# LiWentomng/OrientedRepPoints

Hardware: AMD Instinct MI355X
Metric: images/sec (1024x1024 DOTA, R-50 FPN) (higher is better)
Workload: dtype f32; 1 GPU; configs[1]: OrientedRepPoints R-50 FPN inference, 1024x1024 patch, 15 classes, bs=1/GPU, nms_pre=2000, score_thr=0.05, rnms iou_thr=0.4, max_per_img=2000; random-init weights, head biases calibrated to ~2000 dets/img; global_batch=1, parallelism=replicas x1 (image-parallel, no collective), images_in_flight_per_gpu=4

## Files before the change

include/orp_hip.h:

```cpp
#ifndef ORP_HIP_H_
#define ORP_HIP_H_

#include <stddef.h>
#include <stdint.h>

#ifdef __cplusplus
extern "C" {
#endif

#define ORP_OK 0
#define ORP_EINVAL (-1)
#define ORP_EWORKSPACE (-2)
#define ORP_ETOOBIG (-3)

const char* orp_version(void);

#define ORP_NMS_MAX_BOXES 131072
size_t orp_rnms_workspace_bytes(int n);
int orp_rnms(const float* dets, int n, float iou_thr, int flavor, int presorted, int order_out,
             int64_t* keep_out, int32_t* num_keep, void* workspace, size_t workspace_bytes, void* stream);

size_t orp_rnms_batched_workspace_bytes(int n_total, int nseg, int max_seg);
int orp_rnms_batched(const float* dets, int n_total, const int32_t* seg_offsets, int nseg, int max_seg,
                     float iou_thr, int flavor, int64_t* keep_out, int32_t* num_keep,
// ... 239 lines not shown
int orp_affine2_act(const float* x, const float* residual, const float* scale, const float* shift, const float* scale2,
                    const float* shift2, float* y, int batch, int channels, int hw, int relu, void* stream);
int orp_affine_relu_maxpool(const float* x, const float* scale, const float* shift, float* y, int batch, int channels,
                            int height, int width, void* stream);
size_t orp_affine_act_backward_workspace_bytes(int batch, int channels, int hw);
int orp_affine_act_backward(const float* grad_y, const float* y, const float* x, const float* scale, const float* mean,
                            const float* rstd, float* grad_x, float* grad_res, float* dweight, float* dbias, int batch, int channels,
                            int hw, void* workspace, size_t workspace_bytes, void* stream);
int orp_affine2_act_backward(const float* grad_y, const float* y, const float* x, const float* scale, const float* mean,
                             const float* rstd, const float* x2, const float* scale2, const float* mean2, const float* rstd2,
                             float* grad_x, float* grad_x2, float* grad_res, float* dweight, float* dbias, float* dweight2,
                             float* dbias2, int batch, int channels, int hw, void* workspace, size_t workspace_bytes, void* stream);
size_t orp_fpn_topdown_workspace_bytes(const orp_norm_level* levels, int nlevels, int batch, int channels, int groups);
int orp_fpn_topdown_nhwc(const orp_norm_level* levels, const float* const* gammas_host, const float* const* betas_host,
                         int nlevels, int batch, int channels, int groups, float eps, uint32_t* amax_out, void* workspace,
                         size_t workspace_bytes, void* stream);

typedef struct { const float* input; const float* residual; float* output; float* output2; int height; int width; } orp_bias_level;
int orp_bias_act_multi(const orp_bias_level* levels_host, int nlevels, int batch, int channels, const float* bias,
                       const float* sub, int relu, void* stream);

size_t orp_conv1x1_packed_floats(int c_in);
int orp_conv1x1_ok(int c_in, int c_out);
int orp_conv1x1_pack_weight(const float* weight, int c_out, int c_in, float* packed, void* stream);
int orp_conv1x1_multi(const orp_bias_level* levels_host, int nlevels, int batch, int c_in, int c_out,
                      const float* weight_packed, const float* bias, const float* sub, int relu, void* stream);

int orp_conv1x1_bn_act_ok(int c_in, int c_out);
int orp_conv1x1_bn_act_pays(int c_in, int c_out, int hw, int batch, int has_residual);
int orp_conv1x1_bn_act_tile(int c_in, int c_out, int hw, int batch, int* tile_channels, int* tile_positions);
int orp_conv1x1_bn_act(const float* x, const float* weight_t, const float* scale, const float* shift, const float* residual,
                       const float* scale2, const float* shift2, float* y, int batch, int c_in, int c_out, int hw, int relu,
                       void* stream);

int orp_conv1x1_bn_act_range(const float* x, const float* weight_t, const float* scale, const float* shift, const float* residual,
                             const float* scale2, const float* shift2, float* y, int batch, int c_in, int c_out, int hw, int relu,
                             uint32_t* range_out, void* stream);
int orp_conv1x1_bn_act_pieces_ok(int c_in, int c_out);
int orp_conv1x1_bn_act_pieces_pays(int c_in, int c_out, int hw, int batch, int has_residual);
int orp_conv1x1_bn_act_pieces_tile(int c_in, int c_out, int hw, int batch, int* tile_channels, int* tile_positions);
size_t orp_conv1x1_bn_pieces_packed_bytes(int c_in, int c_out);
int orp_conv1x1_bn_pieces_pack_weight(const float* weight, int c_in, int c_out, void* packed, void* stream);
int orp_conv1x1_bn_act_pieces(const float* x, const void* weight_packed, const float* scale, const float* shift,
                              const float* residual, const float* scale2, const float* shift2, float* y, int batch, int c_in,
                              int c_out, int hw, int relu, uint32_t* range_out, void* stream);

int orp_conv1x1_bn_act_pieces_dual_ok(int c_in, int c_in2, int c_out);
int orp_conv1x1_bn_act_pieces_dual_pays(int c_in, int c_in2, int c_out, int hw, int stride2, int batch);
int orp_conv1x1_bn_act_pieces_dual_tile(int c_in, int c_in2, int c_out, int hw, int batch, int* tile_channels, int* tile_positions);
int orp_conv1x1_bn_act_pieces_dual(const float* x, const void* w_packed, const float* scale, const float* shift, const float* x2,
                                   const void* w2_packed, const float* scale2, const float* shift2, int c_in2, int h2, int w2,
                                   int stride2, float* y, int batch, int c_in, int c_out, int ho, int wo, int relu, void* stream);

int orp_affine_act_range(const float* x, const float* residual, const float* scale, const float* shift, float* y, int batch,
                         int channels, int hw, int relu, uint32_t* range_out, void* stream);

int orp_conv3x3_bn_act_ok(int c_in, int c_out);
int orp_conv3x3_bn_act_pays(int c_in, int c_out, int height, int width, int batch);
int orp_conv3x3_bn_act_tile(int c_in, int c_out, int height, int width, int batch, int* tile_h, int* tile_w, int* waves_pos,
                            int* waves_ch);
size_t orp_conv3x3_bn_packed_bytes(int c_in, int c_out);
int orp_conv3x3_bn_pack_weight(const float* weight, int c_in, int c_out, void* packed, void* stream);
int orp_conv3x3_bn_act(const float* x, const void* weight_packed, const float* scale, const float* shift, const uint32_t* range_in,
                       float* y, int batch, int c_in, int c_out, int height, int width, int relu, void* stream);

int orp_conv3x3_bn_deep_ok(int c_in, int c_out, int stride);
int orp_conv3x3_bn_deep_pays(int c_in, int c_out, int height, int width, int stride, int batch);
size_t orp_conv3x3_bn_deep_packed_bytes(int c_in, int c_out);
int orp_conv3x3_bn_deep_pack_weight(const float* weight, int c_in, int c_out, void* packed, void* stream);
int orp_conv3x3_bn_deep(const float* x, const void* weight_packed, const float* scale, const float* shift, const uint32_t* range_in,
                        float* y, int batch, int c_in, int c_out, int height, int width, int stride, int relu, void* stream);

int orp_conv3x3_bn_s2_ok(int c_in, int c_out);
int orp_conv3x3_bn_s2_pays(int c_in, int c_out, int height, int width, int batch);
size_t orp_conv3x3_bn_s2_packed_bytes(int c_in, int c_out);
int orp_conv3x3_bn_s2_pack_weight(const float* weight, int c_in, int c_out, void* packed, void* stream);
int orp_conv3x3_bn_s2(const float* x, const void* weight_packed, const float* scale, const float* shift, const uint32_t* range_in,
                      float* y, int batch, int c_in, int c_out, int height, int width, int relu, void* stream);

int orp_stem_ok(int c_in, int c_out, int kernel, int stride, int padding);
int orp_stem_pays(int height, int width, int batch);
size_t orp_stem_packed_bytes(int c_in, int c_out);
int orp_stem_pack_weight(const float* weight, int c_in, int c_out, void* packed, void* stream);
int orp_stem_conv_bn_relu_pool(const float* x, const void* weight_packed, const float* scale, const float* shift, float* y, int batch,
                               int c_in, int c_out, int height, int width, int kernel, int stride, int padding, int pool, void* stream);


int orp_conv3x3_small_ok(int c_in, int c_out);
int orp_conv3x3_small_multi(const orp_norm_level* levels_host, int nlevels, int batch, int c_in, int c_out,
                            const float* weight_packed, void* stream);
int orp_conv3x3_small_multi_ex(const orp_norm_level* levels_host, const float* const* weights_packed_host, int nlevels,
                               int batch, int c_in, int c_out, void* stream);
size_t orp_conv3x3_small_workspace_bytes(const orp_norm_level* levels_host, const int* strides_host, int nlevels, int batch,
                                         int c_out);
int orp_conv3x3_small_multi_strided(const orp_norm_level* levels_host, const float* const* weights_packed_host,
                                    const int* strides_host, int nlevels, int batch, int c_in, int c_out, void* workspace,
                                    size_t workspace_bytes, void* stream);

typedef struct { const float* input_a; const float* input_b; float* output_a; float* output_b; int height; int width; } orp_conv_level;
int orp_conv_split_ok(int c_in, int c_out, int kh, int kw);
int orp_conv_split_multi(const orp_conv_level* levels_host, int nlevels, int batch, int c_in, int c_out,
                         const float* weight_a_packed, const float* weight_b_packed, const float* bias_a, const float* bias_b,
                         int relu, int kh, int kw, int stride_h, int stride_w, int pad_h, int pad_w, int dil_h, int dil_w,
                         int out_layout, int nprod, void* workspace, size_t workspace_bytes, const uint32_t* amax_in,
                         int amax_stride, void* stream);
int orp_conv_split_multi_ex(const orp_conv_level* levels_host, const float* const* weights_packed_host,
// ... 88 lines not shown
```

orientedreppoints_amd/build.py:

```python
import concurrent.futures
import os
import subprocess

HERE = os.path.dirname(os.path.abspath(__file__))
CSRC = os.path.join(HERE, "csrc")
LIB = os.path.join(CSRC, "liborp_hip.so")
HIPCC = os.environ.get("HIPCC", "/opt/rocm/bin/hipcc")
ARCH = "gfx950"

NO_PACKED_FP32 = ["-Xclang", "-target-feature", "-Xclang", "-packed-fp32-ops"]
COMMON = ["--offload-arch=" + ARCH, "-O3", "-std=c++17", "-fPIC", "-Wall", "-Wno-unused-function",
          "-Wno-unused-result", "-Wno-unused-value",
          "-Wno-bitwise-instead-of-logical"]
if os.environ.get("ORP_PACKED_FP32", "0") != "1":
    COMMON = COMMON + NO_PACKED_FP32
SOURCES = [
    ("orp_nms.hip", ["-ffp-contract=off"]),
    ("orp_overlaps.hip", ["-ffp-contract=off"]),
    ("orp_minarearect.hip", ["-ffp-contract=off"]),
    ("orp_box_iou_rotated.hip", ["-ffp-contract=off"]),
    ("orp_convex.hip", ["-ffp-contract=off"]),
    ("orp_convex_giou.hip", ["-ffp-contract=off"]),
    ("orp_pointwise.hip", ["-ffp-contract=off"]),
    ("orp_assign.hip", ["-ffp-contract=off"]),
    ("orp_postproc.hip", ["-ffp-contract=off"]),
    ("orp_soft_rnms.hip", ["-ffp-contract=off"]),
    ("orp_scene.hip", ["-ffp-contract=off"]),
    ("orp_train_images.hip", ["-ffp-contract=off"]),
    ("orp_eval.hip", ["-ffp-contract=off"]),
    ("orp_train.hip", ["-ffp-contract=off"]),
    ("orp_norm.hip", []),
    ("orp_conv_small.hip", []),
    ("orp_conv1x1.hip", []),
    ("orp_conv1x1_bn.hip", []),
    ("orp_conv1x1_bn_pieces.hip", []),
    ("orp_conv3x3_bn.hip", []),
    ("orp_conv3x3_bn_deep.hip", []),
    ("orp_conv3x3_bn_s2.hip", []),
    ("orp_stem.hip", []),
    ("orp_dcn.hip", []),
    ("orp_dcn_split.hip", ["-ffp-contract=off"]),
    ("orp_conv_split.hip", []),
    ("orp_conv_wgrad.hip", []),
    ("orp_dcn_half.hip", []),
    ("orp_dcn_bwd.hip", []),
    ("orp_dcn_bwd_mfma.hip", []),
    ("orp_window_attn.hip", []),
    ("orp_token_linear.hip", []),
    ("orp_prof.hip", []),
]
HEADERS = sorted(f for f in os.listdir(CSRC) if f.endswith(".hpp")) + [os.path.join("..", "..", "include", "orp_hip.h")]


def _stale(target, deps):
    if not os.path.exists(target):
        return True
    t = os.path.getmtime(target)
    return any(os.path.getmtime(d) > t for d in deps if os.path.exists(d))


VERSION_SOURCE = "orp_overlaps.hip"


def build_id():
    import hashlib
    h = hashlib.sha1()
    names = sorted([s for s, _ in SOURCES] + [x for x in HEADERS])
    for n in names:
        path = os.path.join(CSRC, n)
        if os.path.exists(path):
            h.update(n.encode())
            h.update(open(path, "rb").read())
    return h.hexdigest()[:12]


def _compile(src, extra):
    obj = os.path.join(CSRC, os.path.splitext(src)[0] + ".o")
    deps = [os.path.join(CSRC, src)] + [os.path.join(CSRC, h) for h in HEADERS] + [os.path.abspath(__file__)]
    if src == VERSION_SOURCE:
        deps += [os.path.join(CSRC, s) for s, _ in SOURCES]
        extra = extra + ['-DORP_BUILD_ID="%s"' % build_id()]
    if _stale(obj, deps):
        cmd = [HIPCC] + COMMON + extra + ["-c", os.path.join(CSRC, src), "-o", obj]
        r = subprocess.run(cmd, cwd=CSRC, stderr=subprocess.PIPE, universal_newlines=True)
        err = "\n".join(l for l in r.stderr.splitlines() if "'-packed-fp32-ops' is not a recognized feature" not in l)
        if err.strip():
            import sys
            sys.stderr.write(err + "\n")
# ... 27 lines not shown
```

orientedreppoints_amd/mmdet_models/resnet.py:

```python
import functools

import torch
import torch.nn as nn

from .. import switches
from .layers import build_conv_layer, build_norm_layer, constant_init, kaiming_init
from .registry import BACKBONES


class Bottleneck(nn.Module):
    expansion = 4

    def __init__(self, inplanes, planes, stride=1, dilation=1, downsample=None, style='pytorch',
                 norm_cfg=dict(type='BN'), dcn=None):
        super(Bottleneck, self).__init__()
        assert style in ['pytorch', 'caffe']
        assert dcn is None or isinstance(dcn, dict)
        if style == 'pytorch':
            conv1_stride, conv2_stride = 1, stride
        else:
            conv1_stride, conv2_stride = stride, 1
        self.conv1 = nn.Conv2d(inplanes, planes, kernel_size=1, stride=conv1_stride, bias=False)
        self.add_module('bn1', build_norm_layer(norm_cfg, planes)[1])
        self.with_dcn = dcn is not None
# ... 19 lines not shown
            isinstance(self.bn1, nn.BatchNorm2d) and not self.bn1.training and not self.bn3.training

    def _norms_are_eval_bn(self):
        return all(isinstance(bn, nn.BatchNorm2d) and not bn.training for bn in (self.bn1, self.bn2, self.bn3)) and \
            (self.downsample is None or self._downsample_is_conv_norm())

    def _frozen_ok(self, x):
        return torch.is_grad_enabled() and not torch.is_autocast_enabled() and x.is_cuda and x.dtype == torch.float32 and \
            not x.requires_grad and not getattr(self, 'with_cp', False) and \
            isinstance(self.bn1, nn.BatchNorm2d) and not self.bn1.training and not self.bn3.training and \
            switches.of(self, 'fuse_bn_frozen', 'BN_FROZEN_FUSE') and not any(p.requires_grad for p in self.parameters())

    def _train_fused_ok(self, x):
        return torch.is_grad_enabled() and not torch.is_autocast_enabled() and x.is_cuda and x.dtype == torch.float32 and \
            x.dim() == 4 and x.is_contiguous() and not getattr(self, 'with_cp', False) and self._norms_are_eval_bn() and \
            switches.of(self, 'fuse_bn_train', 'BN_TRAIN_FUSE')

    def route(self, x):
        if self._fused_ok(x):
            return 'fused'
        if self._frozen_ok(x):
            return 'frozen'
        if self._train_fused_ok(x):
            return 'train'
        return 'stock'

    def _forward_train_fused(self, x):
        from ..mmdet_ops.fused_norm import bn_act_train
        out = bn_act_train(self.conv1(x).contiguous(), self.bn1, relu=True)
        out = bn_act_train(self.conv2(out).contiguous(), self.bn2, relu=True)
        out = self.conv3(out).contiguous()
        ds = self.downsample
        if ds is not None:
            return bn_act_train(out, self.bn3, residual=ds[0](x).contiguous(), residual_bn=ds[1], relu=True)
        return bn_act_train(out, self.bn3, residual=x, relu=True)

    def _downsample_norm_fusable(self):
        return switches.of(self, 'fuse_downsample_norm', 'BN_DOWNSAMPLE_FUSE') and self._downsample_is_conv_norm()

    def _downsample_is_conv_norm(self):
        ds = self.downsample
        return isinstance(ds, nn.Sequential) and len(ds) == 2 and isinstance(ds[0], nn.Conv2d) and \
            isinstance(ds[1], nn.BatchNorm2d) and not ds[1].training

    def _conv1x1_fusable(self):
        return switches.of(self, 'fuse_conv1x1', 'BN_CONV1X1_FUSE')

    def _conv1x1_pieces_on(self):
        return switches.of(self, 'fuse_conv1x1_pieces', 'BN_CONV1X1_PIECES')

    def _downsample_conv_fusable(self):
        return switches.of(self, 'fuse_downsample_conv', 'BN_DOWNSAMPLE_CONV_FUSE')

    def _conv3x3_fusable(self, kind='act'):
        from ..mmdet_ops.fused_norm import conv3x3_kernel
        k = conv3x3_kernel(kind)
        return switches.of(self, k.fuse_attr, k.switch) and not self.conv2_is_dcn and \
            isinstance(self.bn2, nn.BatchNorm2d) and not self.bn2.training

    _conv3x3_deep_fusable = functools.partialmethod(_conv3x3_fusable, 'deep')
    _conv3x3_s2_fusable = functools.partialmethod(_conv3x3_fusable, 's2')

    def _conv3x3_forced(self, kind):
        from ..mmdet_ops.fused_norm import conv3x3_kernel
        return bool(getattr(self, conv3x3_kernel(kind).force_attr, False))

    def _forward_fused(self, x):
        from ..mmdet_ops.fused_norm import bn_act, conv1x1_bn_act, conv3x3_bn_route, _conv3x3_launch, conv1x1_bn_act_dual, \
            conv1x1_bn_act_dual_routed
        fuse = self._conv1x1_fusable()
        pieces = None if self._conv1x1_pieces_on() else False

        def conv_bn_act(t, conv, bn, **kw):
            if fuse:
                return conv1x1_bn_act(t, conv, bn, pieces=pieces, **kw)
            return bn_act(conv(t).contiguous(), bn, **kw)
        kind = None
        if tuple(self.conv1.stride) == (1, 1):
            kind = conv3x3_bn_route(x, self.conv2, self.bn2, (x.size(0), self.conv1.out_channels, x.size(2), x.size(3)),
                                    self._conv3x3_fusable, self._conv3x3_forced)
        if kind is not None:
            out, bits = conv_bn_act(x, self.conv1, self.bn1, relu=True, want_range=True)
            out = _conv3x3_launch(kind, out, self.conv2, self.bn2, relu=True, force=self._conv3x3_forced(kind), range_bits=bits)
        else:
            out = conv_bn_act(x, self.conv1, self.bn1, relu=True)
            out = bn_act(self.conv2(out).contiguous(), self.bn2, relu=True)
        ds = self.downsample
        if fuse and pieces is None and self._downsample_conv_fusable() and self._downsample_is_conv_norm() and \
                conv1x1_bn_act_dual_routed(out, self.conv3, self.bn3, x, ds[0], ds[1]):
            return conv1x1_bn_act_dual(out, self.conv3, self.bn3, x, ds[0], ds[1], relu=True)
        if self._downsample_norm_fusable():
            residual, residual_bn = ds[0](x).contiguous(), ds[1]
        elif ds is not None:
            residual, residual_bn = bn_act(ds[0](x).contiguous(), ds[1], relu=False), None
        else:
            residual, residual_bn = x.contiguous(), None
        return conv_bn_act(out, self.conv3, self.bn3, residual=residual, residual_bn=residual_bn, relu=True)

    def forward(self, x):
        route = self.route(x)
        if route == 'fused':
            return self._forward_fused(x)
        if route == 'frozen':
            with torch.no_grad():
                return self._forward_fused(x)
        if route == 'train':
            return self._forward_train_fused(x)
        identity = x
        out = self.relu(self.bn1(self.conv1(x)))
        out = self.relu(self.bn2(self.conv2(out)))
        out = self.bn3(self.conv3(out))
        if self.downsample is not None:
            identity = self.downsample(x)
        out += identity
        return self.relu(out)


@BACKBONES.register_module
class ResNet(nn.Module):
    arch_settings = {50: (Bottleneck, (3, 4, 6, 3)), 101: (Bottleneck, (3, 4, 23, 3)), 152: (Bottleneck, (3, 8, 36, 3))}

    def __init__(self, depth, in_channels=3, num_stages=4, strides=(1, 2, 2, 2), dilations=(1, 1, 1, 1),
                 out_indices=(0, 1, 2, 3), style='pytorch', frozen_stages=-1, conv_cfg=None,
                 norm_cfg=dict(type='BN', requires_grad=True), norm_eval=True, dcn=None,
                 stage_with_dcn=(False, False, False, False), gcb=None, stage_with_gcb=None, gen_attention=None,
                 stage_with_gen_attention=None, with_cp=False, zero_init_residual=True):
        super(ResNet, self).__init__()
        if depth not in self.arch_settings:
            raise KeyError('invalid depth {} for resnet'.format(depth))
        assert gcb is None and gen_attention is None, 'context / attention blocks are not part of the DOTA configs'
        assert conv_cfg is None, 'the backbone convolutions are stock nn.Conv2d (dcn= selects the deformable conv2)'
        self.dcn = dict(dcn) if dcn is not None else None
        self.stage_with_dcn = tuple(stage_with_dcn) if stage_with_dcn is not None else (False,) * num_stages
        if dcn is not None:
            assert len(self.stage_with_dcn) == num_stages
        self.depth, self.num_stages, self.out_indices = depth, num_stages, out_indices
        self.frozen_stages, self.norm_eval = frozen_stages, norm_eval
        self.zero_init_residual = zero_init_residual
        block, stage_blocks = self.arch_settings[depth]
        self.conv1 = nn.Conv2d(in_channels, 64, kernel_size=7, stride=2, padding=3, bias=False)
        self.add_module('bn1', build_norm_layer(norm_cfg, 64)[1])
        self.relu = nn.ReLU(inplace=True)
        self.maxpool = nn.MaxPool2d(kernel_size=3, stride=2, padding=1)
        inplanes = 64
        self.res_layers = []
        for i, num_blocks in enumerate(stage_blocks[:num_stages]):
            planes = 64 * 2 ** i
            stride, dilation = strides[i], dilations[i]
            downsample = None
            if stride != 1 or inplanes != planes * block.expansion:
                downsample = nn.Sequential(
                    nn.Conv2d(inplanes, planes * block.expansion, kernel_size=1, stride=stride, bias=False),
                    build_norm_layer(norm_cfg, planes * block.expansion)[1])
            stage_dcn = self.dcn if (self.dcn is not None and self.stage_with_dcn[i]) else None
            layers = [block(inplanes, planes, stride, dilation, downsample, style, norm_cfg, stage_dcn)]
            inplanes = planes * block.expansion
            for _ in range(1, num_blocks):
                layers.append(block(inplanes, planes, 1, dilation, None, style, norm_cfg, stage_dcn))
# ... 32 lines not shown
                if missing or unexpected:
                    warnings.warn('ResNet.init_weights(%r): missing keys %s, unexpected keys %s'
                                  % (pretrained, list(missing)[:8], unexpected[:8]))
                return
            warnings.warn('ResNet.init_weights: pretrained=%r was NOT loaded (no such file%s); the backbone keeps its '
                          'random initialisation, frozen_stages=%d of it frozen'
                          % (pretrained, '' if '://' not in pretrained else '; set ORP_PRETRAINED_DIR', self.frozen_stages))
        for m in self.modules():
            if isinstance(m, nn.Conv2d):
                kaiming_init(m)
            elif isinstance(m, (nn.BatchNorm2d, nn.GroupNorm)):
                constant_init(m, 1)
        if self.dcn is not None:
            for m in self.modules():
                if isinstance(m, Bottleneck) and hasattr(m.conv2, 'conv_offset'):
                    constant_init(m.conv2.conv_offset, 0)
        if self.zero_init_residual:
            for m in self.modules():
                if isinstance(m, Bottleneck):
                    constant_init(m.bn3, 0)

    def _stem_pool_fusable(self):
        from ..mmdet_ops.fused_norm import is_maxpool_3_2_1
        return switches.of(self, 'fuse_stem_pool', 'STEM_POOL_FUSE') and is_maxpool_3_2_1(self.maxpool)

    def stem_route(self, x):
        if not (x.is_cuda and x.dtype == torch.float32 and isinstance(self.bn1, nn.BatchNorm2d) and not self.bn1.training):
            return 'stock'
        if not torch.is_grad_enabled():
            return 'fused'
        if not torch.is_autocast_enabled() and not x.requires_grad and switches.of(self, 'fuse_bn_frozen', 'BN_FROZEN_FUSE') and \
                not any(p.requires_grad for m in (self.conv1, self.bn1) for p in m.parameters()):
            return 'frozen'
        return 'stock'

    def _forward_stem_fused(self, x):
        from ..mmdet_ops.fused_norm import bn_act, bn_relu_maxpool, stem_conv_bn_relu_maxpool, stem_conv_routed
        if switches.of(self, 'fuse_stem_conv', 'STEM_CONV_FUSE') and \
                stem_conv_routed(x, self.conv1, self.bn1, self.maxpool, bool(getattr(self, 'force_stem_conv', False))):
            return stem_conv_bn_relu_maxpool(x, self.conv1, self.bn1)
        if self._stem_pool_fusable():
            return bn_relu_maxpool(self.conv1(x).contiguous(), self.bn1)
        return self.maxpool(bn_act(self.conv1(x).contiguous(), self.bn1, relu=True))

    def forward(self, x):
        route = self.stem_route(x)
        if route == 'fused':
            x = self._forward_stem_fused(x)
        elif route == 'frozen':
            with torch.no_grad():
                x = self._forward_stem_fused(x)
        else:
            x = self.maxpool(self.relu(self.bn1(self.conv1(x))))
        outs = []
        for i, name in enumerate(self.res_layers):
            x = getattr(self, name)(x)
            if i in self.out_indices:
                outs.append(x)
        return tuple(outs)

    def train(self, mode=True):
        super(ResNet, self).train(mode)
        self._freeze_stages()
        if mode and self.norm_eval:
            for m in self.modules():
                if isinstance(m, nn.modules.batchnorm._BatchNorm):
                    m.eval()
```

orientedreppoints_amd/mmdet_ops/fused_norm.py:

```python
import collections
import ctypes
import functools

import torch

from .. import _lib, _packcache


_NormLevel = _lib.struct("orp_norm_level")


def _call(name, device, *args):
    with torch.cuda.device(device):
        rc = getattr(_lib.lib(), name)(*args)
    _lib.check(rc, name)


def _norm_levels(ins, outs):
    levels = (_NormLevel * len(ins))()
    for i, (x, y) in enumerate(zip(ins, outs)):
        levels[i] = _NormLevel(x.data_ptr(), y.data_ptr() if y is not None else None, x.size(2), x.size(3))
    return levels


# ... 238 lines not shown
    y = torch.empty((B, cout, H, W), dtype=torch.float32, device=x.device)
    bits = torch.empty(1, dtype=torch.int32, device=x.device) if want_range else None
    args = (_lib.ptr(x), _lib.ptr(weight), _lib.ptr(scale), _lib.ptr(shift), _lib.ptr(residual), _lib.ptr(scale2), _lib.ptr(shift2),
            _lib.ptr(y), B, cin, cout, H * W, 1 if relu else 0)
    if route == 'pieces':
        _call("orp_conv1x1_bn_act_pieces", x.device, *args, _lib.ptr(bits), _lib.stream_of(x))
    elif want_range:
        _call("orp_conv1x1_bn_act_range", x.device, *args, _lib.ptr(bits), _lib.stream_of(x))
    else:
        _call("orp_conv1x1_bn_act", x.device, *args, _lib.stream_of(x))
    return (y, bits) if want_range else y


def conv1x1_bn_act_dual_ok(x, conv, bn, x2, conv2, bn2):
    if not conv1x1_bn_act_ok(x, conv, bn):
        return False
    w2 = getattr(conv2, 'weight', None)
    if not (isinstance(conv2, torch.nn.Conv2d) and _bn_input(x2, bn2) and x2.dim() == 4 and x2.device == x.device and
            _plain_conv(conv2, w2, 1, ((1, 1), (2, 2)), 0) and x2.size(1) == w2.size(1) and
            w2.size(0) == conv.weight.size(0) and x2.size(0) == x.size(0)):
        return False
    s = conv2.stride[0]
    return bool(x2.size(2) > 0 and x2.size(3) > 0 and (x2.size(2) - 1) // s + 1 == x.size(2) and (x2.size(3) - 1) // s + 1 == x.size(3)
                and _lib.lib().orp_conv1x1_bn_act_pieces_dual_ok(conv.weight.size(1), w2.size(1), w2.size(0)))


def conv1x1_bn_act_dual_pays(x, conv, x2, conv2):
    return bool(_lib.lib().orp_conv1x1_bn_act_pieces_dual_pays(conv.weight.size(1), conv2.weight.size(1), conv.weight.size(0),
                                                               x.size(2) * x.size(3), conv2.stride[0], x.size(0)))


def conv1x1_bn_act_dual_routed(x, conv, bn, x2, conv2, bn2):
    return conv1x1_bn_act_dual_ok(x, conv, bn, x2, conv2, bn2) and conv1x1_bn_act_dual_pays(x, conv, x2, conv2)


def conv1x1_bn_act_dual_tile(cin, cin2, cout, hw, B):
    return _tile_query("orp_conv1x1_bn_act_pieces_dual_tile", 2, cin, cin2, cout, hw, B)


def conv1x1_bn_act_dual(x, conv, bn, x2, conv2, bn2, relu=True):
    if not conv1x1_bn_act_dual_ok(x, conv, bn, x2, conv2, bn2):
        raise ValueError("conv1x1_bn_act_dual: unsupported modules or shapes (conv1x1_bn_act_dual_ok)")
    x, x2 = x.detach().contiguous(), x2.detach().contiguous()
    B, cin, H, W = x.shape
    cout, cin2 = conv.weight.size(0), conv2.weight.size(1)
    packed, packed2 = _packed_1x1_planes(conv.weight), _packed_1x1_planes(conv2.weight)
    scale, shift = _bn_affine(bn)
    scale2, shift2 = _bn_affine(bn2)
    y = torch.empty((B, cout, H, W), dtype=torch.float32, device=x.device)
    _call("orp_conv1x1_bn_act_pieces_dual", x.device, _lib.ptr(x), _lib.ptr(packed), _lib.ptr(scale), _lib.ptr(shift), _lib.ptr(x2),
          _lib.ptr(packed2), _lib.ptr(scale2), _lib.ptr(shift2), cin2, x2.size(2), x2.size(3), conv2.stride[0], _lib.ptr(y),
          B, cin, cout, H, W, 1 if relu else 0, _lib.stream_of(x))
    return y


_Conv3x3Kernel = collections.namedtuple("_Conv3x3Kernel", "kind strides ok pays packed_bytes pack_weight launch takes_stride "
                                                           "switch fuse_attr force_attr")
CONV3X3_KERNELS = (
    _Conv3x3Kernel("act", ((1, 1),), "orp_conv3x3_bn_act_ok", "orp_conv3x3_bn_act_pays", "orp_conv3x3_bn_packed_bytes",
                   "orp_conv3x3_bn_pack_weight", "orp_conv3x3_bn_act", False, "BN_CONV3X3_FUSE", "fuse_conv3x3", "force_conv3x3"),
    _Conv3x3Kernel("deep", ((1, 1), (2, 2)), "orp_conv3x3_bn_deep_ok", "orp_conv3x3_bn_deep_pays", "orp_conv3x3_bn_deep_packed_bytes",
                   "orp_conv3x3_bn_deep_pack_weight", "orp_conv3x3_bn_deep", True, "BN_CONV3X3_DEEP_FUSE", "fuse_conv3x3_deep",
                   "force_conv3x3_deep"),
    _Conv3x3Kernel("s2", ((2, 2),), "orp_conv3x3_bn_s2_ok", "orp_conv3x3_bn_s2_pays", "orp_conv3x3_bn_s2_packed_bytes",
                   "orp_conv3x3_bn_s2_pack_weight", "orp_conv3x3_bn_s2", False, "BN_CONV3X3_S2_FUSE", "fuse_conv3x3_s2", "force_conv3x3_s2"),
)
_CONV3X3 = {k.kind: k for k in CONV3X3_KERNELS}


def conv3x3_kernel(kind):
    return _CONV3X3[kind]


def _stride_arg(k, conv):
    return (conv.stride[0],) if k.takes_stride else ()


def _conv3x3_ok(kind, x, conv, bn, shape=None):
    k = _CONV3X3[kind]
    w = getattr(conv, 'weight', None)
    shape = tuple(x.shape) if shape is None else tuple(shape)
    return bool(type(conv) is torch.nn.Conv2d and _bn_input(x, bn) and len(shape) == 4 and
                _plain_conv(conv, w, 3, k.strides, 1) and shape[1] == w.size(1) and shape[0] * shape[2] * shape[3] > 0 and
                getattr(_lib.lib(), k.ok)(w.size(1), w.size(0), *_stride_arg(k, conv)))


def _conv3x3_routed(kind, x, conv, bn, force=False, shape=None):
    if not _conv3x3_ok(kind, x, conv, bn, shape):
        return False
    k = _CONV3X3[kind]
    B, _c, H, W = tuple(x.shape) if shape is None else tuple(shape)
    return bool(force or getattr(_lib.lib(), k.pays)(conv.weight.size(1), conv.weight.size(0), H, W, *_stride_arg(k, conv), B))


def conv3x3_bn_route(x, conv, bn, shape, enabled, forced):
    for k in CONV3X3_KERNELS:
        if enabled(k.kind) and _conv3x3_routed(k.kind, x, conv, bn, forced(k.kind), shape):
            return k.kind
    return None


_packed_3x3_cache = _packcache.new_cache("conv3x3_bn_weight")


def _packed_3x3(kind, weight):
    k = _CONV3X3[kind]
# ... 800 lines not shown
```

orientedreppoints_amd/switches.py:

```python
import os


def _on(name, default='1'):
    return os.environ.get(name, default) == '1'


TOWER_SPLIT = _on('ORP_TOWER_SPLIT')
FPN_SPLIT = _on('ORP_FPN_SPLIT')
TOWER_GN_FUSE = _on('ORP_TOWER_GN_FUSE')
BN_DOWNSAMPLE_FUSE = _on('ORP_BN_DOWNSAMPLE_FUSE')
BN_CONV1X1_FUSE = _on('ORP_BN_CONV1X1_FUSE')
BN_CONV1X1_PIECES = _on('ORP_BN_CONV1X1_PIECES')
BN_DOWNSAMPLE_CONV_FUSE = _on('ORP_BN_DOWNSAMPLE_CONV_FUSE')
BN_CONV3X3_FUSE = _on('ORP_BN_CONV3X3_FUSE')
BN_CONV3X3_DEEP_FUSE = _on('ORP_BN_CONV3X3_DEEP_FUSE')
BN_CONV3X3_S2_FUSE = _on('ORP_BN_CONV3X3_S2_FUSE')
BN_TRAIN_FUSE = _on('ORP_BN_TRAIN_FUSE')
BN_FROZEN_FUSE = _on('ORP_BN_FROZEN_FUSE')
STEM_POOL_FUSE = _on('ORP_STEM_POOL_FUSE')
STEM_CONV_FUSE = _on('ORP_STEM_CONV_FUSE')
SWIN_ATTN_FUSE = _on('ORP_SWIN_ATTN_FUSE')
SWIN_ATTN_TRAIN_FUSE = _on('ORP_SWIN_ATTN_TRAIN_FUSE')
SWIN_ATTN_HALF_FUSE = _on('ORP_SWIN_ATTN_HALF_FUSE')
SWIN_LINEAR_FUSE = _on('ORP_SWIN_LINEAR_FUSE')
FPN_TOPDOWN_FUSE = _on('ORP_FPN_TOPDOWN_FUSE')
TRAIN_SPLIT = _on('ORP_TRAIN_SPLIT')
DETERMINISTIC = _on('ORP_DETERMINISTIC', '0')


def of(obj, attr, name):
    on = getattr(obj, attr, None)
    return bool(globals()[name] if on is None else on)
```

Baseline: 468.0 images/s.

## Fuse bottleneck conv3 with next block's conv1 in one chained 1x1 kernel

Adds a HIP kernel that computes a bottleneck's final 1x1 conv+BN+residual+ReLU and immediately feeds the result tile from LDS into the next block's first 1x1 conv+BN+ReLU, writing both outputs. The ResNet forward links consecutive Bottleneck blocks so the next block reuses the handed-off conv1 output and range bits. This removes one kernel launch and the re-read of the wide intermediate from global memory for the second conv. It is gated by a pays table covering only the 128->512->128 stage-2 shape at hw=16384, batch 1. It adds per-forward Python bookkeeping and a new MFMA kernel with a heavier LDS and register footprint.

```diff
diff --git a/include/orp_hip.h b/include/orp_hip.h
--- a/include/orp_hip.h
+++ b/include/orp_hip.h
@@ -315,6 +315,14 @@
                                    const void* w2_packed, const float* scale2, const float* shift2, int c_in2, int h2, int w2,
                                    int stride2, float* y, int batch, int c_in, int c_out, int ho, int wo, int relu, void* stream);
 
+int orp_conv1x1_bn_act_pieces_chain_ok(int c_in, int c_out, int c_next);
+int orp_conv1x1_bn_act_pieces_chain_pays(int c_in, int c_out, int c_next, int hw, int batch);
+int orp_conv1x1_bn_act_pieces_chain_tile(int c_in, int c_out, int c_next, int hw, int batch, int* tile_channels, int* tile_positions);
+int orp_conv1x1_bn_act_pieces_chain(const float* x, const void* w_packed, const float* scale, const float* shift, const float* residual,
+                                    float* y, const void* w_next_packed, const float* scale_next, const float* shift_next, float* t,
+                                    int batch, int c_in, int c_out, int c_next, int hw, int relu, int relu_next, uint32_t* range_out,
+                                    void* stream);
+
 int orp_affine_act_range(const float* x, const float* residual, const float* scale, const float* shift, float* y, int batch,
                          int channels, int hw, int relu, uint32_t* range_out, void* stream);
 
diff --git a/orientedreppoints_amd/build.py b/orientedreppoints_amd/build.py
--- a/orientedreppoints_amd/build.py
+++ b/orientedreppoints_amd/build.py
@@ -34,6 +34,7 @@
     ("orp_conv1x1.hip", []),
     ("orp_conv1x1_bn.hip", []),
     ("orp_conv1x1_bn_pieces.hip", []),
+    ("orp_conv1x1_bn_chain.hip", []),
     ("orp_conv3x3_bn.hip", []),
     ("orp_conv3x3_bn_deep.hip", []),
     ("orp_conv3x3_bn_s2.hip", []),
diff --git a/orientedreppoints_amd/csrc/orp_conv1x1_bn_chain.hip b/orientedreppoints_amd/csrc/orp_conv1x1_bn_chain.hip
--- /dev/null
+++ b/orientedreppoints_amd/csrc/orp_conv1x1_bn_chain.hip
@@ -0,0 +1,372 @@
+#include <hip/hip_runtime.h>
+#include <stdint.h>
+
+#include "../../include/orp_hip.h"
+#include "orp_affine.hpp"
+#include "orp_range.hpp"
+#include "orp_launch.hpp"
+#include "orp_conv1x1_bn_host.hpp"
+#include "orp_dcn_split.hpp"
+
+namespace {
+
+constexpr int kThreads = 256;
+constexpr int kTileCh = 128;
+constexpr int kMaxCout = 1024;
+
+typedef float f32x16 __attribute__((ext_vector_type(16)));
+typedef __bf16 bf8 __attribute__((ext_vector_type(8)));
+
+struct ChainArgs {
+  const float* x;
+  const uint16_t* planes;
+  size_t plane_stride;
+  const float* scale; const float* shift;
+  const float* res;
+  float* y;
+  const uint16_t* planes2;
+  size_t plane_stride2;
+  const float* scale2; const float* shift2;
+  float* t;
+  int cout, hw, relu, relu2;
+  int ntn;
+  int vec;
+  unsigned* range;
+};
+
+using orp_split::split_pair;
+
+__device__ __forceinline__ void six(f32x16& acc, const bf8 (&w)[3], const bf8 (&x)[3]) {
+  acc = __builtin_amdgcn_mfma_f32_32x32x16_bf16(w[0], x[2], acc, 0, 0, 0);
+  acc = __builtin_amdgcn_mfma_f32_32x32x16_bf16(w[2], x[0], acc, 0, 0, 0);
+  acc = __builtin_amdgcn_mfma_f32_32x32x16_bf16(w[1], x[1], acc, 0, 0, 0);
+  acc = __builtin_amdgcn_mfma_f32_32x32x16_bf16(w[0], x[1], acc, 0, 0, 0);
+  acc = __builtin_amdgcn_mfma_f32_32x32x16_bf16(w[1], x[0], acc, 0, 0, 0);
+  acc = __builtin_amdgcn_mfma_f32_32x32x16_bf16(w[0], x[0], acc, 0, 0, 0);
+}
+
+constexpr size_t chain_lds_bytes(int cin, int bn) {
+  return (size_t)3 * bn * (cin + 8 + kTileCh + 8) * 2 + (size_t)2 * kTileCh * 4;
+}
+
+template <int CIN, int CNEXT, int WN>
+__global__ void __launch_bounds__(kThreads, 2)
+conv1x1_bn_chain_kernel(const ChainArgs P) {
+  constexpr int BN = 32 * WN;
+  constexpr int XSTR = CIN + 8, YSTR = kTileCh + 8;
+  constexpr int XPLANE = BN * XSTR, YPLANE = BN * YSTR;
+  constexpr int NCH = CIN / 16;
+  constexpr int NCH2 = kTileCh / 16;
+  constexpr int WCH2 = CNEXT >= 128 ? 4 : 2, WPOS2 = 4 / WCH2;
+  constexpr int MT2 = CNEXT / (32 * WCH2), NT2 = WN / WPOS2;
+  static_assert(NT2 >= 1 && MT2 >= 1, "Cnext = 64 needs 64 positions");
+  constexpr int D1 = MT2 * NT2 >= 4 ? 2 : 3;
+  constexpr int D2 = MT2 == 1 ? 4 : 2;
+  constexpr int ITEMS = (CIN / 2) * (BN / 4);
+  constexpr int XV = ITEMS / kThreads;
+  static_assert(ITEMS % kThreads == 0, "whole trips");
+
+  extern __shared__ __align__(16) uint16_t lds[];
+  uint16_t* Xs = lds;
+  uint16_t* Ys = lds + 3 * XPLANE;
+  float* Cs = reinterpret_cast<float*>(Ys + 3 * YPLANE);
+
+  const int tid = threadIdx.x;
+  const int nt = blockIdx.x % P.ntn, b = blockIdx.x / P.ntn;
+  const int p0 = nt * BN;
+  const int hw = P.hw, cout = P.cout;
+  const float* xb = P.x + (size_t)b * CIN * hw;
+
+  const int lane = tid & 63, wave = tid >> 6;
+  const int kg = lane >> 5, l31 = lane & 31;
+
+  const size_t plane0 = (size_t)b * cout;
+  float rv[WN][16];
+  auto load_res = [&](int m0) {
+#pragma unroll
+    for (int ni = 0; ni < WN; ni++) {
+      const int p = min(p0 + 32 * ni + l31, hw - 1);
+#pragma unroll
+      for (int r = 0; r < 16; r++) {
+        const int ch = m0 + 32 * wave + 8 * (r >> 2) + 4 * kg + (r & 3);
+        rv[ni][r] = P.res[(plane0 + ch) * hw + p];
+      }
+    }
+  };
+
+  {
+    float4 xr[XV][2];
+#pragma unroll
+    for (int i = 0; i < XV; i++) {
+      const int idx = tid + i * kThreads;
+      const int pq = idx % (BN / 4), kp = idx / (BN / 4);
+      const int col = p0 + 4 * pq;
+#pragma unroll
+      for (int h = 0; h < 2; h++) {
+        const float* src = xb + (size_t)(2 * kp + h) * hw;
+        if (P.vec) {
+          xr[i][h] = *reinterpret_cast<const float4*>(src + min(col, hw - 4));
+        } else {
+          xr[i][h].x = src[min(col, hw - 1)]; xr[i][h].y = src[min(col + 1, hw - 1)];
+          xr[i][h].z = src[min(col + 2, hw - 1)]; xr[i][h].w = src[min(col + 3, hw - 1)];
+        }
+      }
+    }
+#pragma unroll
+    for (int i = 0; i < XV; i++) {
+      const int idx = tid + i * kThreads;
+      const int pq = idx % (BN / 4), kp = idx / (BN / 4);
+      const int col = p0 + 4 * pq;
+      float v[2][4];
+#pragma unroll
+      for (int h = 0; h < 2; h++) {
+        v[h][0] = col < hw ? xr[i][h].x : 0.f; v[h][1] = col + 1 < hw ? xr[i][h].y : 0.f;
+        v[h][2] = col + 2 < hw ? xr[i][h].z : 0.f; v[h][3] = col + 3 < hw ? xr[i][h].w : 0.f;
+      }
+      const int rot = (pq >> 1) & 3;
+#pragma unroll
+      for (int h = 0; h < 2; h++) {
+        if (rot & 1) { const float t0 = v[h][0]; v[h][0] = v[h][1]; v[h][1] = v[h][2]; v[h][2] = v[h][3]; v[h][3] = t0; }
+        if (rot & 2) { const float t0 = v[h][0], t1 = v[h][1]; v[h][0] = v[h][2]; v[h][1] = v[h][3]; v[h][2] = t0; v[h][3] = t1; }
+      }
+      unsigned* base = reinterpret_cast<unsigned*>(Xs) + kp;
+#pragma unroll
+      for (int j = 0; j < 4; j++) {
+        unsigned d[3];
+        split_pair(v[0][j], v[1][j], d);
+        unsigned* dst = base + (4 * pq + ((j + rot) & 3)) * (XSTR / 2);
+#pragma unroll
+        for (int pl = 0; pl < 3; pl++) dst[pl * (XPLANE / 2)] = d[pl];
+      }
+    }
+  }
+
+  const size_t ps = P.plane_stride, ps2 = P.plane_stride2;
+  const size_t wblk = (size_t)2 * cout * 8, wblk2 = (size_t)2 * CNEXT * 8;
+  const uint16_t* wp = P.planes + ((size_t)kg * cout + 32 * wave + l31) * 8;
+  const int wc2 = (wave / WPOS2) * 32 * MT2, wn2 = (wave % WPOS2) * 32 * NT2;
+  const uint16_t* wp2 = P.planes2 + ((size_t)kg * CNEXT + wc2 + l31) * 8;
+  bf8 wq[NCH][3], w2q[NCH2][MT2][3];
+  auto load_w = [&](int m0, int c) {
+    const uint16_t* a = wp + (size_t)m0 * 8 + (size_t)c * wblk;
+#pragma unroll
+    for (int pl = 0; pl < 3; pl++) wq[c][pl] = *reinterpret_cast<const bf8*>(a + (size_t)pl * ps);
+  };
+  auto load_w2 = [&](int chunk0, int c) {
+    const uint16_t* a = wp2 + (size_t)(chunk0 + c) * wblk2;
+#pragma unroll
+    for (int mi = 0; mi < MT2; mi++)
+#pragma unroll
+      for (int pl = 0; pl < 3; pl++) w2q[c][mi][pl] = *reinterpret_cast<const bf8*>(a + (size_t)pl * ps2 + (size_t)mi * 32 * 8);
+  };
+
+  f32x16 tacc[MT2][NT2];
+#pragma unroll
+  for (int mi = 0; mi < MT2; mi++)
+#pragma unroll
+    for (int ni = 0; ni < NT2; ni++)
+#pragma unroll
+      for (int r = 0; r < 16; r++) tacc[mi][ni][r] = 0.f;
+
+#pragma unroll
+  for (int c = 0; c < D1; c++) load_w(0, c);
+  __syncthreads();
+
+  const int ntm = cout / kTileCh;
+  const uint16_t* xa = Xs + l31 * XSTR + 8 * kg;
+  const uint16_t* ya = Ys + (wn2 + l31) * YSTR + 8 * kg;
+  for (int mt = 0; mt < ntm; mt++) {
+    const int m0 = mt * kTileCh;
+    if (tid < kTileCh) { Cs[tid] = P.scale[m0 + tid]; Cs[kTileCh + tid] = P.shift[m0 + tid]; }
+    load_res(m0);
+    f32x16 acc[WN];
+#pragma unroll
+    for (int ni = 0; ni < WN; ni++)
+#pragma unroll
+      for (int r = 0; r < 16; r++) acc[ni][r] = 0.f;
+    __builtin_amdgcn_sched_barrier(0);
+
+#pragma unroll
+    for (int c = 0; c < NCH; c++) {
+      bf8 xq[WN][3];
+#pragma unroll
+      for (int ni = 0; ni < WN; ni++)
+#pragma unroll
+        for (int pl = 0; pl < 3; pl++) xq[ni][pl] = *reinterpret_cast<const bf8*>(xa + pl * XPLANE + ni * 32 * XSTR + c * 16);
+#pragma unroll
+      for (int ni = 0; ni < WN; ni++) six(acc[ni], wq[c], xq[ni]);
+      __builtin_amdgcn_sched_barrier(0);
+      if (c + D1 < NCH) load_w(m0, c + D1);
+      __builtin_amdgcn_sched_barrier(0);
+    }
+#pragma unroll
+    for (int c = 0; c < D2; c++) load_w2(mt * NCH2, c);
+    __builtin_amdgcn_sched_barrier(0);
+    __syncthreads();
+
+#pragma unroll
+    for (int g = 0; g < 4; g++) {
+      const int chl = 32 * wave + 8 * g + 4 * kg;
+      const float4 a4 = *reinterpret_cast<const float4*>(Cs + chl);
+      const float4 b4 = *reinterpret_cast<const float4*>(Cs + kTileCh + chl);
+      const float av[4] = {a4.x, a4.y, a4.z, a4.w}, bv[4] = {b4.x, b4.y, b4.z, b4.w};
+#pragma unroll
+      for (int ni = 0; ni < WN; ni++) {
+        const int pl_ = 32 * ni + l31, p = p0 + pl_;
+        float v[4];
+#pragma unroll
+        for (int q = 0; q < 4; q++) {
+          v[q] = affine_res_act(acc[ni][4 * g + q], av[q], bv[q], rv[ni][4 * g + q], P.relu);
+          if (p < hw) P.y[(plane0 + m0 + chl + q) * hw + p] = v[q];
+        }
+        unsigned d0[3], d1[3];
+        split_pair(v[0], v[1], d0);
+        split_pair(v[2], v[3], d1);
+        uint2* dst = reinterpret_cast<uint2*>(Ys + pl_ * YSTR + chl);
+#pragma unroll
+        for (int pl = 0; pl < 3; pl++) dst[pl * (YPLANE / 4)] = make_uint2(d0[pl], d1[pl]);
+      }
+    }
+    __builtin_amdgcn_sched_barrier(0);
+#pragma unroll
+    for (int c = 0; c < D1; c++) load_w(min(mt + 1, ntm - 1) * kTileCh, c);
+    __syncthreads();
+
+#pragma unroll
+    for (int c = 0; c < NCH2; c++) {
+      bf8 yq[NT2][3];
+#pragma unroll
+      for (int ni = 0; ni < NT2; ni++)
+#pragma unroll
+        for (int pl = 0; pl < 3; pl++) yq[ni][pl] = *reinterpret_cast<const bf8*>(ya + pl * YPLANE + ni * 32 * YSTR + c * 16);
+#pragma unroll
+      for (int mi = 0; mi < MT2; mi++)
+#pragma unroll
+        for (int ni = 0; ni < NT2; ni++) six(tacc[mi][ni], w2q[c][mi], yq[ni]);
+      __builtin_amdgcn_sched_barrier(0);
+      if (c + D2 < NCH2) load_w2(mt * NCH2, c + D2);
+      __builtin_amdgcn_sched_barrier(0);
+    }
+  }
+
+  unsigned rmax = 0u;
+  const size_t tplane0 = (size_t)b * CNEXT;
+#pragma unroll
+  for (int mi = 0; mi < MT2; mi++)
+#pragma unroll
+    for (int g = 0; g < 4; g++) {
+      const int ch = wc2 + 32 * mi + 8 * g + 4 * kg;
+      float av[4], bv[4];
+#pragma unroll
+      for (int q = 0; q < 4; q++) { av[q] = P.scale2[ch + q]; bv[q] = P.shift2[ch + q]; }
+#pragma unroll
+      for (int ni = 0; ni < NT2; ni++) {
+        const int p = p0 + wn2 + 32 * ni + l31;
+#pragma unroll
+        for (int q = 0; q < 4; q++) {
+          const float v = affine_act(tacc[mi][ni][4 * g + q], av[q], bv[q], P.relu2);
+          if (p < hw) {
+            P.t[(tplane0 + ch + q) * hw + p] = v;
+            rmax = max(rmax, orp::range_bits(v));
+          }
+        }
+      }
+    }
+  if (P.range) {
+#pragma unroll
+    for (int o = 32; o > 0; o >>= 1) rmax = max(rmax, (unsigned)__shfl_xor((int)rmax, o, 64));
+    unsigned* red = reinterpret_cast<unsigned*>(lds);
+    __syncthreads();
+    if (lane == 0) red[wave] = rmax;
+    __syncthreads();
+    if (tid == 0) orp::range_raise(P.range, max(max(red[0], red[1]), max(red[2], red[3])));
+  }
+}
+
+int pick_bn(int c_next, int hw, int batch) {
+  if (c_next < 128) return 64;
+  return (long)((hw + 63) / 64) * batch >= 256 ? 64 : 32;
+}
+
+template <int CIN, int CNEXT, int WN>
+hipError_t launch(const ChainArgs& A, int batch, hipStream_t st) {
+  const size_t smem = chain_lds_bytes(CIN, 32 * WN);
+  struct Tag {};
+  hipError_t e = orp::set_max_dynamic_lds_once<Tag>(reinterpret_cast<const void*>(&conv1x1_bn_chain_kernel<CIN, CNEXT, WN>), smem);
+  if (e != hipSuccess) return e;
+  hipLaunchKernelGGL((conv1x1_bn_chain_kernel<CIN, CNEXT, WN>), dim3((unsigned)((long)A.ntn * batch)), dim3(kThreads), smem, st, A);
+  return hipGetLastError();
+}
+
+bool overlap(const void* a, size_t na, const void* b, size_t nb) {
+  const uintptr_t x = (uintptr_t)a, y = (uintptr_t)b;
+  return x < y + nb && y < x + na;
+}
+
+}
+
+extern "C" {
+
+int orp_conv1x1_bn_act_pieces_chain_ok(int c_in, int c_out, int c_next) {
+  const bool pair = (c_in == 64 && (c_next == 64 || c_next == 128)) || (c_in == 128 && (c_next == 128 || c_next == 256));
+  return (pair && c_out >= kTileCh && c_out <= kMaxCout && c_out % kTileCh == 0) ? 1 : 0;
+}
+
+int orp_conv1x1_bn_act_pieces_chain_tile(int c_in, int c_out, int c_next, int hw, int batch, int* tile_channels, int* tile_positions) {
+  if (!orp_conv1x1_bn_act_pieces_chain_ok(c_in, c_out, c_next) || hw <= 0 || batch <= 0) return 0;
+  if (tile_channels) *tile_channels = c_out;
+  if (tile_positions) *tile_positions = pick_bn(c_next, hw, batch);
+  return 1;
+}
+
+int orp_conv1x1_bn_act_pieces_chain_pays(int c_in, int c_out, int c_next, int hw, int batch) {
+  if (!orp_conv1x1_bn_act_pieces_chain_ok(c_in, c_out, c_next) || hw <= 0 || batch <= 0) return 0;
+  if (!orp_conv1x1_bn_act_pieces_pays(c_in, c_out, hw, batch, 1) || !orp_conv1x1_bn_act_pieces_pays(c_out, c_next, hw, batch, 0)) return 0;
+  static const struct { int cin, cout, cnext, hw_min, hw_max, batch; } paid[] = {
+      {128, 512, 128, 16384, 16384, 1},
+  };
+  for (const auto& s : paid)
+    if (s.cin == c_in && s.cout == c_out && s.cnext == c_next && s.batch == batch && hw >= s.hw_min && hw <= s.hw_max) return 1;
+  return 0;
+}
+
+int orp_conv1x1_bn_act_pieces_chain(const float* x, const void* w_packed, const float* scale, const float* shift, const float* residual,
+                                    float* y, const void* w_next_packed, const float* scale_next, const float* shift_next, float* t,
+                                    int batch, int c_in, int c_out, int c_next, int hw, int relu, int relu_next, uint32_t* range_out,
+                                    void* stream) {
+  if (!x || !w_packed || !scale || !shift || !residual || !y || !w_next_packed || !scale_next || !shift_next || !t || batch <= 0 ||
+      hw <= 0 || !orp_conv1x1_bn_act_pieces_chain_ok(c_in, c_out, c_next))
+    return ORP_EINVAL;
+  if (((uintptr_t)w_packed & 15) || ((uintptr_t)w_next_packed & 15)) return ORP_EINVAL;
+  if ((long)hw >= (1L << 31) / 4) return ORP_ETOOBIG;
+  const int bn = pick_bn(c_next, hw, batch);
+  const long ntn = (hw + bn - 1) / bn;
+  if (ntn * batch >= (1L << 31)) return ORP_ETOOBIG;
+  const size_t nx = (size_t)batch * c_in * hw * 4, ny = (size_t)batch * c_out * hw * 4, nt_ = (size_t)batch * c_next * hw * 4;
+  if (overlap(y, ny, x, nx) || overlap(y, ny, residual, ny) || overlap(t, nt_, x, nx) || overlap(t, nt_, residual, ny) ||
+      overlap(t, nt_, y, ny))
+    return ORP_EINVAL;
+  if (range_out && (overlap(range_out, 4, y, ny) || overlap(range_out, 4, t, nt_))) return ORP_EINVAL;
+  ChainArgs A{};
+  A.x = x; A.planes = reinterpret_cast<const uint16_t*>(w_packed); A.plane_stride = (size_t)c_in * c_out;
+  A.scale = scale; A.shift = shift; A.res = residual; A.y = y;
+  A.planes2 = reinterpret_cast<const uint16_t*>(w_next_packed); A.plane_stride2 = (size_t)c_out * c_next;
+  A.scale2 = scale_next; A.shift2 = shift_next; A.t = t;
+  A.cout = c_out; A.hw = hw; A.relu = relu ? 1 : 0; A.relu2 = relu_next ? 1 : 0;
+  A.ntn = (int)ntn; A.vec = ((hw & 3) == 0 && ((uintptr_t)x & 15) == 0) ? 1 : 0;
+  A.range = range_out;
+  hipStream_t st = (hipStream_t)stream;
+  if (range_out) {
+    hipError_t fe = orp::fill_async(range_out, 0, sizeof(uint32_t), st);
+    if (fe != hipSuccess) return (int)fe;
+  }
+  hipError_t e;
+  const bool wide = bn == 64;
+  if (c_in == 64 && c_next == 64) e = launch<64, 64, 2>(A, batch, st);
+  else if (c_in == 64) e = wide ? launch<64, 128, 2>(A, batch, st) : launch<64, 128, 1>(A, batch, st);
+  else if (c_next == 128) e = wide ? launch<128, 128, 2>(A, batch, st) : launch<128, 128, 1>(A, batch, st);
+  else e = wide ? launch<128, 256, 2>(A, batch, st) : launch<128, 256, 1>(A, batch, st);
+  return e == hipSuccess ? ORP_OK : (int)e;
+}
+
+}
diff --git a/orientedreppoints_amd/mmdet_models/resnet.py b/orientedreppoints_amd/mmdet_models/resnet.py
--- a/orientedreppoints_amd/mmdet_models/resnet.py
+++ b/orientedreppoints_amd/mmdet_models/resnet.py
@@ -95,6 +95,25 @@
     def _downsample_conv_fusable(self):
         return switches.of(self, 'fuse_downsample_conv', 'BN_DOWNSAMPLE_CONV_FUSE')
 
+    def _conv1x1_chain_on(self):
+        return switches.of(self, 'fuse_conv1x1_chain', 'BN_CONV1X1_CHAIN')
+
+    def _chain_candidate(self, x):
+        nxt = getattr(self, '_chain_next', None)
+        nxt = nxt[0] if nxt else None
+        if not (isinstance(nxt, Bottleneck) and self._conv1x1_chain_on() and nxt._conv1x1_chain_on()):
+            return None
+        if self.conv2_is_dcn or nxt.conv2_is_dcn or tuple(nxt.conv1.stride) != (1, 1) or nxt.route(x) not in ('fused', 'frozen'):
+            return None
+        return nxt
+
+    def _chains_into(self, nxt, out, residual, fuse, pieces):
+        from ..mmdet_ops.fused_norm import conv1x1_bn_act_chain_routed
+        if nxt is None or not fuse or pieces is False or not (nxt._conv1x1_fusable() and nxt._conv1x1_pieces_on()):
+            return False
+        force = bool(getattr(self, 'force_conv1x1_chain', False)) and bool(getattr(nxt, 'force_conv1x1_chain', False))
+        return conv1x1_bn_act_chain_routed(out, self.conv3, self.bn3, residual, nxt.conv1, nxt.bn1, force=force)
+
     def _conv3x3_fusable(self, kind='act'):
         from ..mmdet_ops.fused_norm import conv3x3_kernel
         k = conv3x3_kernel(kind)
@@ -108,11 +127,15 @@
         from ..mmdet_ops.fused_norm import conv3x3_kernel
         return bool(getattr(self, conv3x3_kernel(kind).force_attr, False))
 
-    def _forward_fused(self, x):
+    def _forward_fused(self, x, nxt=None):
         from ..mmdet_ops.fused_norm import bn_act, conv1x1_bn_act, conv3x3_bn_route, _conv3x3_launch, conv1x1_bn_act_dual, \
-            conv1x1_bn_act_dual_routed
+            conv1x1_bn_act_dual_routed, conv1x1_bn_act_chain
         fuse = self._conv1x1_fusable()
         pieces = None if self._conv1x1_pieces_on() else False
+        if pieces is None and getattr(self, 'force_conv1x1_chain', False):
+            pieces = True
+        handed = self.__dict__.pop('_chain_in', None)
+        handed = handed if handed is not None and handed[0] is x else None
 
         def conv_bn_act(t, conv, bn, **kw):
             if fuse:
@@ -123,10 +146,10 @@
             kind = conv3x3_bn_route(x, self.conv2, self.bn2, (x.size(0), self.conv1.out_channels, x.size(2), x.size(3)),
                                     self._conv3x3_fusable, self._conv3x3_forced)
         if kind is not None:
-            out, bits = conv_bn_act(x, self.conv1, self.bn1, relu=True, want_range=True)
+            out, bits = handed[1:] if handed is not None else conv_bn_act(x, self.conv1, self.bn1, relu=True, want_range=True)
             out = _conv3x3_launch(kind, out, self.conv2, self.bn2, relu=True, force=self._conv3x3_forced(kind), range_bits=bits)
         else:
-            out = conv_bn_act(x, self.conv1, self.bn1, relu=True)
+            out = handed[1] if handed is not None else conv_bn_act(x, self.conv1, self.bn1, relu=True)
             out = bn_act(self.conv2(out).contiguous(), self.bn2, relu=True)
         ds = self.downsample
         if fuse and pieces is None and self._downsample_conv_fusable() and self._downsample_is_conv_norm() and \
@@ -138,15 +161,21 @@
             residual, residual_bn = bn_act(ds[0](x).contiguous(), ds[1], relu=False), None
         else:
             residual, residual_bn = x.contiguous(), None
+            if self._chains_into(nxt, out, residual, fuse, pieces):
+                y, t, bits = conv1x1_bn_act_chain(out, self.conv3, self.bn3, residual, nxt.conv1, nxt.bn1, want_range=True)
+                nxt.__dict__['_chain_in'] = (y, t, bits)
+                return y
         return conv_bn_act(out, self.conv3, self.bn3, residual=residual, residual_bn=residual_bn, relu=True)
 
     def forward(self, x):
         route = self.route(x)
         if route == 'fused':
-            return self._forward_fused(x)
+            return self._forward_fused(x, self._chain_candidate(x))
         if route == 'frozen':
+            nxt = self._chain_candidate(x)
             with torch.no_grad():
-                return self._forward_fused(x)
+                return self._forward_fused(x, nxt)
+        self.__dict__.pop('_chain_in', None)
         if route == 'train':
             return self._forward_train_fused(x)
         identity = x
@@ -285,11 +314,23 @@
                 x = self._forward_stem_fused(x)
         else:
             x = self.maxpool(self.relu(self.bn1(self.conv1(x))))
+        stages = [getattr(self, name) for name in self.res_layers]
+        blocks = [m if isinstance(m, Bottleneck) else None
+                  for s in stages for m in (s if isinstance(s, nn.Sequential) else [None])]
+        for a, b in zip(blocks[:-1], blocks[1:]):
+            if a is not None and b is not None:
+                a.__dict__['_chain_next'] = (b,)
+        blocks = [m for m in blocks if m is not None]
         outs = []
-        for i, name in enumerate(self.res_layers):
-            x = getattr(self, name)(x)
-            if i in self.out_indices:
-                outs.append(x)
+        try:
+            for i, name in enumerate(self.res_layers):
+                x = getattr(self, name)(x)
+                if i in self.out_indices:
+                    outs.append(x)
+        finally:
+            for m in blocks:
+                m.__dict__.pop('_chain_next', None)
+                m.__dict__.pop('_chain_in', None)
         return tuple(outs)
 
     def train(self, mode=True):
diff --git a/orientedreppoints_amd/mmdet_ops/fused_norm.py b/orientedreppoints_amd/mmdet_ops/fused_norm.py
--- a/orientedreppoints_amd/mmdet_ops/fused_norm.py
+++ b/orientedreppoints_amd/mmdet_ops/fused_norm.py
@@ -314,6 +314,50 @@
           _lib.ptr(packed2), _lib.ptr(scale2), _lib.ptr(shift2), cin2, x2.size(2), x2.size(3), conv2.stride[0], _lib.ptr(y),
           B, cin, cout, H, W, 1 if relu else 0, _lib.stream_of(x))
     return y
+
+
+def conv1x1_bn_act_chain_ok(x, conv, bn, residual, conv_next, bn_next):
+    if not conv1x1_bn_act_ok(x, conv, bn):
+        return False
+    w, wn = conv.weight, getattr(conv_next, 'weight', None)
+    if not (isinstance(residual, torch.Tensor) and residual.device == x.device and residual.dtype == torch.float32 and
+            tuple(residual.shape) == (x.size(0), w.size(0), x.size(2), x.size(3)) and residual.is_contiguous()):
+        return False
+    return bool(isinstance(conv_next, torch.nn.Conv2d) and isinstance(bn_next, torch.nn.BatchNorm2d) and not bn_next.training and
+                _plain_conv(conv_next, wn, 1, ((1, 1),), 0) and wn.size(1) == w.size(0) and wn.device == w.device and
+                _lib.lib().orp_conv1x1_bn_act_pieces_chain_ok(w.size(1), w.size(0), wn.size(0)))
+
+
+def conv1x1_bn_act_chain_pays(x, conv, conv_next):
+    return bool(_lib.lib().orp_conv1x1_bn_act_pieces_chain_pays(conv.weight.size(1), conv.weight.size(0), conv_next.weight.size(0),
+                                                                x.size(2) * x.size(3), x.size(0)))
+
+
+def conv1x1_bn_act_chain_routed(x, conv, bn, residual, conv_next, bn_next, force=False):
+    return conv1x1_bn_act_chain_ok(x, conv, bn, residual, conv_next, bn_next) and \
+        (bool(force) or conv1x1_bn_act_chain_pays(x, conv, conv_next))
+
+
+def conv1x1_bn_act_chain_tile(cin, cout, cnext, hw, B):
+    return _tile_query("orp_conv1x1_bn_act_pieces_chain_tile", 2, cin, cout, cnext, hw, B)
+
+
+def conv1x1_bn_act_chain(x, conv, bn, residual, conv_next, bn_next, want_range=False, relu=True, relu_next=True):
+    if not conv1x1_bn_act_chain_ok(x, conv, bn, residual, conv_next, bn_next):
+        raise ValueError("conv1x1_bn_act_chain: unsupported modules or shapes (conv1x1_bn_act_chain_ok)")
+    x, residual = x.detach().contiguous(), residual.detach()
+    B, cin, H, W = x.shape
+    cout, cnext = conv.weight.size(0), conv_next.weight.size(0)
+    packed, packed_next = _packed_1x1_planes(conv.weight), _packed_1x1_planes(conv_next.weight)
+    scale, shift = _bn_affine(bn)
+    scale_next, shift_next = _bn_affine(bn_next)
+    y = torch.empty((B, cout, H, W), dtype=torch.float32, device=x.device)
+    t = torch.empty((B, cnext, H, W), dtype=torch.float32, device=x.device)
+    bits = torch.empty(1, dtype=torch.int32, device=x.device) if want_range else None
+    _call("orp_conv1x1_bn_act_pieces_chain", x.device, _lib.ptr(x), _lib.ptr(packed), _lib.ptr(scale), _lib.ptr(shift),
+          _lib.ptr(residual), _lib.ptr(y), _lib.ptr(packed_next), _lib.ptr(scale_next), _lib.ptr(shift_next), _lib.ptr(t),
+          B, cin, cout, cnext, H * W, 1 if relu else 0, 1 if relu_next else 0, _lib.ptr(bits), _lib.stream_of(x))
+    return (y, t, bits) if want_range else (y, t)
 
 
 _Conv3x3Kernel = collections.namedtuple("_Conv3x3Kernel", "kind strides ok pays packed_bytes pack_weight launch takes_stride "
diff --git a/orientedreppoints_amd/switches.py b/orientedreppoints_amd/switches.py
--- a/orientedreppoints_amd/switches.py
+++ b/orientedreppoints_amd/switches.py
@@ -12,6 +12,7 @@
 BN_CONV1X1_FUSE = _on('ORP_BN_CONV1X1_FUSE')
 BN_CONV1X1_PIECES = _on('ORP_BN_CONV1X1_PIECES')
 BN_DOWNSAMPLE_CONV_FUSE = _on('ORP_BN_DOWNSAMPLE_CONV_FUSE')
+BN_CONV1X1_CHAIN = _on('ORP_BN_CONV1X1_CHAIN')
 BN_CONV3X3_FUSE = _on('ORP_BN_CONV3X3_FUSE')
 BN_CONV3X3_DEEP_FUSE = _on('ORP_BN_CONV3X3_DEEP_FUSE')
 BN_CONV3X3_S2_FUSE = _on('ORP_BN_CONV3X3_S2_FUSE')
```

Result: no change. 463.6 images/s (-0.9%).
